# iamgroot42/A-LINK

Measured on AMD Instinct MI355X. Metric: 112x112 face embeddings/sec (IR-ResNet-100 ArcFace, 512-d, L2-normalised), higher is better.
Workload: dtype bf16

## Files before the change

a-link_amd/csrc/conv_igemm.hip:

```cpp
#include "conv_device.h"

namespace alink {

namespace {

template <typename T, int WP, int WC, bool DMA, bool SP>
__global__ __launch_bounds__(256, 2) void conv_igemm_kernel(const ConvParams p) {
    typedef typename Vec8<T>::type vec8;
    constexpr int BM = WP * 64, BN = WC * 64;
    constexpr int PJ = BM / 32, WJ = BN / 32;
    constexpr int TILE_BYTES = (BM + BN) * 128;
    extern __shared__ __attribute__((aligned(16))) char smem[];

    const int tid  = threadIdx.x;
    const int lane = tid & 63;
    const int wave = __builtin_amdgcn_readfirstlane(tid >> 6);
    const int wp = wave / WC, wc = wave % WC;

    const int ntn = p.Cout / BN;
    const int nwg = gridDim.x;
    const int lid = xcd_remap(blockIdx.x, nwg);
    const int tile_n = lid % ntn, tile_m = lid / ntn;
    const int m0 = tile_m * BM, n0 = tile_n * BN;
    const int split = blockIdx.y;

    const int Cin = p.Cin, W = p.W, ksz = p.ksz;
    const int CinP = SP ? 2 * Cin : Cin;
    const int Cin2 = SP ? 0 : p.Cin2;
    const int K = (SP ? 2 : 1) * ksz * ksz * Cin + Cin2;
    const int cpt = Cin >> 6;
    const int cpt2 = Cin2 >> 6;
    const int ntap = ksz * ksz;
    const int nk = ntap * cpt * (SP ? 3 : 1) + cpt2;
    const int kt0 = split * p.ksteps_per_split;
    const int kt1 = min(kt0 + p.ksteps_per_split, nk);

    const T* __restrict__ gin = (const T*)p.in;
    const T* __restrict__ gin2 = (const T*)p.in2;
    const T* __restrict__ gw  = (const T*)p.wgt;
    const T* __restrict__ gz  = (const T*)p.zero;

    const int chunk = (tid & 7) ^ ((tid >> 4) & 7);
    int      poff[PJ], poff2[PJ];
    unsigned pmask[PJ];
    {
        const int HoWo = p.Ho * p.Wo;
#pragma unroll
        for (int j = 0; j < PJ; ++j) {
            const int m = m0 + (tid >> 3) + 32 * j;
            unsigned mask = 0;
            int off = 0;
            poff2[j] = -1;
            if (m < p.M) {
                const int n = m / HoWo, rem = m - n * HoWo;
                const int oy = rem / p.Wo, ox = rem - oy * p.Wo;
                const int iy0 = oy * p.stride - p.pad, ix0 = ox * p.stride - p.pad;
                off = ((n * p.H + iy0) * W + ix0) * CinP + chunk * 8;
                poff2[j] = (p.in2_compact ? m : (n * p.H + oy * p.stride) * W + ox * p.stride) * Cin2 + chunk * 8;
                for (int ky = 0; ky < ksz; ++ky)
                    for (int kx = 0; kx < ksz; ++kx)
                        if ((unsigned)(iy0 + ky) < (unsigned)p.H && (unsigned)(ix0 + kx) < (unsigned)W)
                            mask |= 1u << (ky * ksz + kx);
            }
            poff[j] = off;
            pmask[j] = mask;
        }
    }
    int woff[WJ];
#pragma unroll
    for (int j = 0; j < WJ; ++j) woff[j] = (n0 + (tid >> 3) + 32 * j) * K + chunk * 8;

    const int r0 = SP ? kt0 / 3 : kt0;
    int s_ph = SP ? kt0 - 3 * r0 : 0;
    int s_tap = r0 / cpt, s_cc = r0 - s_tap * cpt;
    int s_ky = s_tap / ksz, s_kx = s_tap - s_ky * ksz;

    auto stage = [&](int buf, int kt) {
        char* base = smem + buf * TILE_BYTES;
        const int tap_off = (s_ky * W + s_kx) * CinP + (SP ? 2 * s_cc + (s_ph == 2 ? 1 : 0) : s_cc) * 64;
        const int wk_off = SP ? ((s_tap * cpt + s_cc) * 2 + (s_ph == 1 ? 1 : 0)) * 64 : kt * 64;
        const bool shortcut = !SP && s_tap == ntap;
#pragma unroll
        for (int j = 0; j < PJ; ++j) {
            const bool ok = shortcut ? poff2[j] >= 0 : (pmask[j] >> s_tap) & 1u;
            const T* src = ok ? (shortcut ? gin2 + (poff2[j] + s_cc * 64) : gin + (poff[j] + tap_off)) : gz + (tid & 7) * 8;
            if constexpr (DMA) {
                dma16(src, base + (wave * 8 + 32 * j) * 128);
            } else {
                *(uint4*)(base + ((tid >> 3) + 32 * j) * 128 + (tid & 7) * 16) = *(const uint4*)src;
            }
        }
        char* wbase = base + BM * 128;
#pragma unroll
        for (int j = 0; j < WJ; ++j) {
            const T* src = gw + (woff[j] + wk_off);
            if constexpr (DMA) {
                dma16(src, wbase + (wave * 8 + 32 * j) * 128);
            } else {
                *(uint4*)(wbase + ((tid >> 3) + 32 * j) * 128 + (tid & 7) * 16) = *(const uint4*)src;
            }
        }
        if (SP && ++s_ph < 3) return;
        s_ph = 0;
        if (++s_cc == (shortcut ? cpt2 : cpt)) {
            s_cc = 0;
            ++s_tap;
            if (++s_kx == ksz) { s_kx = 0; ++s_ky; }
        }
    };

    const int q = lane >> 4, lr = lane & 15;
    const int sw = lr >> 1;
    const int foff0 = lr * 128 + (((0 | q) ^ sw) << 4);
    const int foff1 = lr * 128 + (((4 | q) ^ sw) << 4);

    f32x4 acc[4][4];
#pragma unroll
    for (int t = 0; t < 4; ++t)
#pragma unroll
        for (int u = 0; u < 4; ++u) acc[t][u] = f32x4{0.f, 0.f, 0.f, 0.f};

    auto mma = [&](const char* pb, const char* wb) {
#pragma unroll
        for (int ks = 0; ks < 2; ++ks) {
            const int fo = ks ? foff1 : foff0;
            vec8 wf[4], pf[4];
#pragma unroll
            for (int t = 0; t < 4; ++t) wf[t] = *(const vec8*)(wb + t * 2048 + fo);
#pragma unroll
            for (int u = 0; u < 4; ++u) pf[u] = *(const vec8*)(pb + u * 2048 + fo);
#pragma unroll
            for (int t = 0; t < 4; ++t)
#pragma unroll
                for (int u = 0; u < 4; ++u) acc[t][u] = mfma16<T>(wf[t], pf[u], acc[t][u]);
        }
    };
    if constexpr (SP) {
        char* const A0 = smem, * const W0 = smem + BM * 128, * const A1 = smem + TILE_BYTES, * const W1 = smem + TILE_BYTES + BM * 128;
        auto stage_a = [&](char* dst, int part) {
            const int tap_off = (s_ky * W + s_kx) * CinP + (2 * s_cc + part) * 64;
#pragma unroll
            for (int j = 0; j < PJ; ++j) {
                const bool ok = (pmask[j] >> s_tap) & 1u;
                dma16(ok ? gin + (poff[j] + tap_off) : gz + (tid & 7) * 8, dst + (wave * 8 + 32 * j) * 128);
            }
        };
        auto stage_w = [&](char* dst, int blk) {
            const int wk_off = ((s_tap * cpt + s_cc) * 2 + blk) * 64;
#pragma unroll
            for (int j = 0; j < WJ; ++j) dma16(gw + (woff[j] + wk_off), dst + (wave * 8 + 32 * j) * 128);
        };
        auto advance = [&]() {
            if (++s_cc == cpt) {
                s_cc = 0;
                ++s_tap;
                if (++s_kx == ksz) { s_kx = 0; ++s_ky; }
            }
        };
        const int r1 = kt1 / 3;
        if (p.nprod == 1) {
            if (r0 < r1) {
                stage_a(A1, 0);
                stage_w(W0, 0);
                __syncthreads();
                for (int r = r0; r < r1; ++r) {
                    const bool odd = (r - r0) & 1;
                    advance();
                    if (r + 1 < r1) {
                        stage_a(odd ? A1 : A0, 0);
                        stage_w(odd ? W0 : W1, 0);
                    }
                    mma((odd ? A0 : A1) + (wp * 64) * 128, (odd ? W1 : W0) + (wc * 64) * 128);
                    __syncthreads();
                }
            }
        } else
        if (r0 < r1) {
            stage_a(A0, 1);
            stage_w(W0, 0);
            __syncthreads();
            const char* const pa0 = A0 + (wp * 64) * 128, * const pa1 = A1 + (wp * 64) * 128;
            const char* const pw0 = W0 + (wc * 64) * 128, * const pw1 = W1 + (wc * 64) * 128;
            for (int r = r0; r < r1; ++r) {
                stage_a(A1, 0);
                mma(pa0, pw0);
                __syncthreads();
                stage_w(W1, 1);
                mma(pa1, pw0);
                __syncthreads();
                advance();
                if (r + 1 < r1) {
                    stage_a(A0, 1);
                    stage_w(W0, 0);
                }
                mma(pa1, pw1);
                __syncthreads();
            }
        }
    } else
    if (kt0 < kt1) {
        stage(0, kt0);
        __syncthreads();
        for (int kt = kt0; kt < kt1; ++kt) {
            const int cur = (kt - kt0) & 1;
            if (kt + 1 < kt1) stage(cur ^ 1, kt + 1);
            mma(smem + cur * TILE_BYTES + (wp * 64) * 128, smem + cur * TILE_BYTES + (BM + wc * 64) * 128);
            __syncthreads();
        }
    }

    const int cbase = n0 + wc * 64 + 16 * q;
    if (p.splitk > 1) {
        float* slab = (float*)p.out + (size_t)split * p.M * p.Cout;
#pragma unroll
        for (int u = 0; u < 4; ++u) {
            const int m = m0 + wp * 64 + 16 * u + lr;
            if (m < p.M) {
                float* o = slab + (size_t)m * p.Cout + cbase;
#pragma unroll
                for (int t = 0; t < 4; ++t) *(f32x4*)(o + 4 * t) = acc[t][u];
            }
        }
        return;
    }

    const int HoWo = p.Ho * p.Wo;
    size_t off[4];
    bool ok[4];
    int cls[4];
#pragma unroll
    for (int u = 0; u < 4; ++u) {
        const int m = m0 + wp * 64 + 16 * u + lr;
        ok[u] = m < p.M;
        const int mc = ok[u] ? m : p.M - 1;
        off[u] = SP ? (size_t)mc * (2 * p.Cout) + (size_t)(cbase >> 6) * 128 + (cbase & 63) : (size_t)mc * p.Cout + cbase;
        cls[u] = 0;
        if (p.border_cls) {
            const int rem = mc % HoWo;
            const int oy = rem / p.Wo, ox = rem - oy * p.Wo;
            const int rc = (oy == 0) ? 0 : ((oy == p.Ho - 1) ? 2 : 1);
            const int cc = (ox == 0) ? 0 : ((ox == p.Wo - 1) ? 2 : 1);
            cls[u] = rc * 3 + cc;
        }
    }
    vec8 res[4][SP ? 4 : 2];
    const T* extra = (const T*)(p.dact ? p.dact : p.resid);
    if (extra) {
#pragma unroll
        for (int u = 0; u < 4; ++u) {
            res[u][0] = *(const vec8*)(extra + off[u]);
            res[u][1] = *(const vec8*)(extra + off[u] + 8);
            if (SP) {
                res[u][2] = *(const vec8*)(extra + off[u] + 64);
                res[u][3] = *(const vec8*)(extra + off[u] + 72);
            }
        }
    }
    f32x4 bia[4][4];
#pragma unroll
    for (int u = 0; u < 4; ++u)
#pragma unroll
        for (int t = 0; t < 4; ++t) bia[u][t] = *(const f32x4*)(p.bias + cls[u] * p.Cout + cbase + 4 * t);
    float al[16];
    if (p.alpha) {
#pragma unroll
        for (int t = 0; t < 4; ++t) {
            const f32x4 a4 = *(const f32x4*)(p.alpha + cbase + 4 * t);
#pragma unroll
            for (int j = 0; j < 4; ++j) al[4 * t + j] = a4[j];
        }
    }
#pragma unroll
    for (int u = 0; u < 4; ++u) {
        float v[16];
#pragma unroll
        for (int t = 0; t < 4; ++t)
#pragma unroll
            for (int j = 0; j < 4; ++j)
                v[4 * t + j] = SP ? fmaf(acc[t][u][j], p.acc_scale, bia[u][t][j] * p.bias_scale) : acc[t][u][j] + bia[u][t][j];
        if (!SP && p.dact) {
#pragma unroll
            for (int i = 0; i < 8; ++i) {
                v[i] *= (float)res[u][0][i] > 0.f ? 1.f : al[i];
                v[8 + i] *= (float)res[u][1][i] > 0.f ? 1.f : al[8 + i];
            }
        } else {
            if (p.alpha) {
#pragma unroll
                for (int i = 0; i < 16; ++i) v[i] = v[i] > 0.f ? v[i] : v[i] * al[i];
            }
            if (p.resid) {
#pragma unroll
                for (int i = 0; i < 8; ++i) {
                    if (SP) {
                        v[i] = fmaf((float)res[u][0][i] + (float)res[u][2][i], p.res_scale, v[i]);
                        v[8 + i] = fmaf((float)res[u][1][i] + (float)res[u][3][i], p.res_scale, v[8 + i]);
                    } else {
                        v[i] += (float)res[u][0][i];
                        v[8 + i] += (float)res[u][1][i];
                    }
                }
            }
        }
        if (p.post_relu) {
#pragma unroll
            for (int i = 0; i < 16; ++i) v[i] = relu_keep_nan(v[i]);
        }
        if (ok[u]) {
            vec8 o0, o1;
#pragma unroll
            for (int i = 0; i < 8; ++i) {
                o0[i] = (T)v[i];
                o1[i] = (T)v[8 + i];
            }
            *(vec8*)((T*)p.out + off[u]) = o0;
            *(vec8*)((T*)p.out + off[u] + 8) = o1;
            if (SP) {
                vec8 l0, l1;
#pragma unroll
                for (int i = 0; i < 8; ++i) {
                    l0[i] = (T)(v[i] - (float)o0[i]);
                    l1[i] = (T)(v[8 + i] - (float)o1[i]);
                }
                *(vec8*)((T*)p.out + off[u] + 64) = l0;
                *(vec8*)((T*)p.out + off[u] + 72) = l1;
            }
        }
    }
}

template <typename T, int WP, int WC, bool DMA, bool SP = false>
hipError_t launch_one(const ConvParams& p, hipStream_t stream) {
    constexpr int BM = WP * 64, BN = WC * 64;
    constexpr size_t lds = 2 * (size_t)(BM + BN) * 128;
    const int ntm = (p.M + BM - 1) / BM, ntn = p.Cout / BN;
    dim3 grid(ntm * ntn, p.splitk, 1), block(256, 1, 1);
    hipLaunchKernelGGL((conv_igemm_kernel<T, WP, WC, DMA, SP>), grid, block, lds, stream, p);
    return hipGetLastError();
}

template <typename T, int WP, int WC, bool DMA, bool SP = false>
hipError_t set_attr_one() {
    constexpr size_t lds = 2 * (size_t)(WP * 64 + WC * 64) * 128;
    return hipFuncSetAttribute((const void*)conv_igemm_kernel<T, WP, WC, DMA, SP>,
                               hipFuncAttributeMaxDynamicSharedMemorySize, (int)lds);
}

bool g_use_dma = true;

}

extern "C" void alink_debug_set_dma(int on) { g_use_dma = on != 0; }

hipError_t conv_set_attributes() {
    hipError_t e;
#define A(T, WP, WC)                                                    \
    if ((e = set_attr_one<T, WP, WC, true>()) != hipSuccess) return e;  \
    if ((e = set_attr_one<T, WP, WC, false>()) != hipSuccess) return e;
    A(__bf16, 4, 1) A(__bf16, 2, 2) A(_Float16, 4, 1) A(_Float16, 2, 2)
#undef A
    if ((e = set_attr_one<_Float16, 4, 1, true, true>()) != hipSuccess) return e;
    if ((e = set_attr_one<_Float16, 2, 2, true, true>()) != hipSuccess) return e;
    return hipSuccess;
}

double conv_flops(const ConvParams& p) {
    return 2.0 * (double)p.M * (double)p.Cout * (double)(p.ksz * p.ksz * p.Cin + (p.in2 ? p.Cin2 : 0));
}

hipError_t launch_conv_igemm(int dtype, const ConvParams& p, hipStream_t stream) {
    if (p.Cin % 64 || p.Cout % 64 || p.M <= 0 || p.splitk < 1) return hipErrorInvalidValue;
    if (p.in2 ? (p.Cin2 <= 0 || p.Cin2 % 64 || p.splitk != 1 || dtype == ALINK_DT_F16X2) : p.Cin2 != 0) return hipErrorInvalidValue;
    if ((long long)p.N * p.H * p.W * p.Cin2 >= (1ll << 31)) return hipErrorInvalidValue;
    if (p.ksz * p.ksz > 32) return hipErrorInvalidValue;
    const int two = dtype == ALINK_DT_F16X2 ? 2 : 1;
    if ((long long)p.N * p.H * p.W * p.Cin * two >= (1ll << 31)) return hipErrorInvalidValue;
    if ((long long)p.Cout * p.ksz * p.ksz * p.Cin * two >= (1ll << 31)) return hipErrorInvalidValue;
    if (conv_gemm_lat_applies(dtype, p)) return launch_conv_gemm_lat(dtype, p, stream);
    const bool wide = (p.Cout % 128) == 0;
    if (dtype == ALINK_DT_F16X2) {
        if (p.dact || (p.splitk > 1 && p.ksteps_per_split % 3)) return hipErrorInvalidValue;
        return wide ? launch_one<_Float16, 2, 2, true, true>(p, stream) : launch_one<_Float16, 4, 1, true, true>(p, stream);
    }
#define L(T)                                                                          \
    (wide ? (g_use_dma ? launch_one<T, 2, 2, true>(p, stream)                         \
                       : launch_one<T, 2, 2, false>(p, stream))                       \
          : (g_use_dma ? launch_one<T, 4, 1, true>(p, stream)                         \
                       : launch_one<T, 4, 1, false>(p, stream)))
    if (dtype == ALINK_DT_BF16) return L(__bf16);
    if (dtype == ALINK_DT_F16) return L(_Float16);
#undef L
    return hipErrorInvalidValue;
}

}
```

include/alink_hip_debug.h:

```cpp
#ifndef ALINK_HIP_DEBUG_H
#define ALINK_HIP_DEBUG_H

#include <stddef.h>

#ifdef __cplusplus
extern "C" {
#endif

void alink_debug_set_linear(int mode);
void alink_debug_set_generic_epilogue(int on);
void alink_debug_set_direct(int on);
void alink_debug_set_pair(int on);
void alink_debug_set_c64(int on);
void alink_debug_set_s2direct(int on);
void alink_debug_set_fuse_stem(int on);
void alink_debug_set_fuse_unit(int mode);
void alink_debug_set_fuse_unit1(int mode);
void alink_debug_set_fuse_shortcut(int on);
void alink_debug_set_dma(int on);
void alink_debug_set_fine_max(int n);
void alink_debug_set_sibling_aware(int on);
void alink_debug_set_latency_form(int max_pixels);
void alink_debug_set_latency_tiles(int form);
void alink_debug_set_stagger(int n);
void alink_debug_set_early_refill(int on);
void alink_debug_set_shard_stagger(int on);

void alink_debug_set_tiny_step(int on);
void alink_debug_set_mini_step(int on);
void alink_debug_set_head_bf16_mfma(int on);

void alink_debug_set_smallres_overlap(int on);
void alink_debug_set_smallres_one_update(int on);

void alink_debug_set_stop_after(int n);
void alink_debug_set_profile_reps(int n);
void alink_debug_set_ablate(int a);
void alink_debug_set_stamps(void* dev_u64);
int alink_debug_lds_oob_probe(float* dev_out516, void* stream);
int alink_debug_linear_contract_ok(void);


struct alink_resnet50;
struct alink_backbone;
int alink_debug_resnet50_grad_cache_info(const struct alink_resnet50* r, int n_images, int index, size_t* byte_offset, int* H,
                                         int* W, int* C, char* name_buf, int name_len);
int alink_debug_backbone_grad_cache_info(const struct alink_backbone* bb, int n_images, int index, size_t* byte_offset, int* H,
                                         int* W, int* C, char* name_buf, int name_len);

#ifdef __cplusplus
}
#endif
#endif
```

Baseline: 50460.

## Add eight-wave wide-tile implicit-GEMM conv kernel with three-stage LDS pipeline

Adds a 512-thread conv kernel with 128x256 or 256x128 tiles and a configurable two- or three-stage LDS pipeline using async DMA with counted waits. It is chosen by default for Cout divisible by 256 when the grid still covers the compute units, aiming to raise operand reuse per workgroup and hide global load latency. The epilogue is factored into a templated helper with a specialised plain variant that drops unused bias-class, residual and activation logic. Optional per-block timing stamps are added too. The risks are lower occupancy (one workgroup per CU, large LDS use) and fewer workgroups on small layers.

```diff
diff --git a/a-link_amd/csrc/conv_igemm.hip b/a-link_amd/csrc/conv_igemm.hip
--- a/a-link_amd/csrc/conv_igemm.hip
+++ b/a-link_amd/csrc/conv_igemm.hip
@@ -3,6 +3,9 @@
 namespace alink {
 
 namespace {
+
+template <typename T, bool SP, int EPI>
+__device__ __forceinline__ void igemm_epilogue(const ConvParams& p, const f32x4 (&acc)[4][4], int mrow0, int cbase, int lr, int split);
 
 template <typename T, int WP, int WC, bool DMA, bool SP>
 __global__ __launch_bounds__(256, 2) void conv_igemm_kernel(const ConvParams p) {
@@ -23,6 +26,9 @@
     const int tile_n = lid % ntn, tile_m = lid / ntn;
     const int m0 = tile_m * BM, n0 = tile_n * BN;
     const int split = blockIdx.y;
+    unsigned long long* const stamps = (SP || p.splitk > 1) ? nullptr : (unsigned long long*)p.stamps;
+    unsigned long long wait_cycles = 0;
+    if (stamps && tid == 0) stamps[(size_t)blockIdx.x * 8 + 0] = __builtin_amdgcn_s_memtime();
 
     const int Cin = p.Cin, W = p.W, ksz = p.ksz;
     const int CinP = SP ? 2 * Cin : Cin;
@@ -201,20 +207,40 @@
     if (kt0 < kt1) {
         stage(0, kt0);
         __syncthreads();
+        if (stamps && tid == 0) stamps[(size_t)blockIdx.x * 8 + 1] = __builtin_amdgcn_s_memtime();
         for (int kt = kt0; kt < kt1; ++kt) {
             const int cur = (kt - kt0) & 1;
             if (kt + 1 < kt1) stage(cur ^ 1, kt + 1);
             mma(smem + cur * TILE_BYTES + (wp * 64) * 128, smem + cur * TILE_BYTES + (BM + wc * 64) * 128);
-            __syncthreads();
-        }
-    }
-
-    const int cbase = n0 + wc * 64 + 16 * q;
-    if (p.splitk > 1) {
+            if (stamps) {
+                asm volatile("s_waitcnt lgkmcnt(0)" ::: "memory");
+                const unsigned long long t0 = __builtin_amdgcn_s_memtime();
+                __syncthreads();
+                wait_cycles += __builtin_amdgcn_s_memtime() - t0;
+            } else {
+                __syncthreads();
+            }
+        }
+    }
+
+    if (stamps && tid == 0) stamps[(size_t)blockIdx.x * 8 + 2] = __builtin_amdgcn_s_memtime();
+    igemm_epilogue<T, SP, 0>(p, acc, m0 + wp * 64, n0 + wc * 64 + 16 * q, lr, split);
+    if (stamps && tid == 0) {
+        asm volatile("s_waitcnt vmcnt(0)" ::: "memory");
+        stamps[(size_t)blockIdx.x * 8 + 3] = __builtin_amdgcn_s_memtime();
+        stamps[(size_t)blockIdx.x * 8 + 4] = wait_cycles;
+        stamps[(size_t)blockIdx.x * 8 + 5] = (unsigned long long)(kt1 - kt0);
+    }
+}
+
+template <typename T, bool SP, int EPI>
+__device__ __forceinline__ void igemm_epilogue(const ConvParams& p, const f32x4 (&acc)[4][4], int mrow0, int cbase, int lr, int split) {
+    typedef typename Vec8<T>::type vec8;
+    if (EPI == 0 && p.splitk > 1) {
         float* slab = (float*)p.out + (size_t)split * p.M * p.Cout;
 #pragma unroll
         for (int u = 0; u < 4; ++u) {
-            const int m = m0 + wp * 64 + 16 * u + lr;
+            const int m = mrow0 + 16 * u + lr;
             if (m < p.M) {
                 float* o = slab + (size_t)m * p.Cout + cbase;
 #pragma unroll
@@ -230,12 +256,12 @@
     int cls[4];
 #pragma unroll
     for (int u = 0; u < 4; ++u) {
-        const int m = m0 + wp * 64 + 16 * u + lr;
+        const int m = mrow0 + 16 * u + lr;
         ok[u] = m < p.M;
         const int mc = ok[u] ? m : p.M - 1;
         off[u] = SP ? (size_t)mc * (2 * p.Cout) + (size_t)(cbase >> 6) * 128 + (cbase & 63) : (size_t)mc * p.Cout + cbase;
         cls[u] = 0;
-        if (p.border_cls) {
+        if (EPI == 0 && p.border_cls) {
             const int rem = mc % HoWo;
             const int oy = rem / p.Wo, ox = rem - oy * p.Wo;
             const int rc = (oy == 0) ? 0 : ((oy == p.Ho - 1) ? 2 : 1);
@@ -244,7 +270,7 @@
         }
     }
     vec8 res[4][SP ? 4 : 2];
-    const T* extra = (const T*)(p.dact ? p.dact : p.resid);
+    const T* extra = EPI == 0 ? (const T*)(p.dact ? p.dact : p.resid) : nullptr;
     if (extra) {
 #pragma unroll
         for (int u = 0; u < 4; ++u) {
@@ -261,8 +287,9 @@
     for (int u = 0; u < 4; ++u)
 #pragma unroll
         for (int t = 0; t < 4; ++t) bia[u][t] = *(const f32x4*)(p.bias + cls[u] * p.Cout + cbase + 4 * t);
+    const bool prelu = EPI == 0 && p.alpha;
     float al[16];
-    if (p.alpha) {
+    if (prelu) {
 #pragma unroll
         for (int t = 0; t < 4; ++t) {
             const f32x4 a4 = *(const f32x4*)(p.alpha + cbase + 4 * t);
@@ -278,18 +305,18 @@
 #pragma unroll
             for (int j = 0; j < 4; ++j)
                 v[4 * t + j] = SP ? fmaf(acc[t][u][j], p.acc_scale, bia[u][t][j] * p.bias_scale) : acc[t][u][j] + bia[u][t][j];
-        if (!SP && p.dact) {
+        if (EPI == 0 && !SP && p.dact) {
 #pragma unroll
             for (int i = 0; i < 8; ++i) {
                 v[i] *= (float)res[u][0][i] > 0.f ? 1.f : al[i];
                 v[8 + i] *= (float)res[u][1][i] > 0.f ? 1.f : al[8 + i];
             }
         } else {
-            if (p.alpha) {
+            if (prelu) {
 #pragma unroll
                 for (int i = 0; i < 16; ++i) v[i] = v[i] > 0.f ? v[i] : v[i] * al[i];
             }
-            if (p.resid) {
+            if (EPI == 0 && p.resid) {
 #pragma unroll
                 for (int i = 0; i < 8; ++i) {
                     if (SP) {
@@ -302,7 +329,7 @@
                 }
             }
         }
-        if (p.post_relu) {
+        if (EPI == 0 && p.post_relu) {
 #pragma unroll
             for (int i = 0; i < 16; ++i) v[i] = relu_keep_nan(v[i]);
         }
@@ -326,6 +353,169 @@
                 *(vec8*)((T*)p.out + off[u] + 72) = l1;
             }
         }
+    }
+}
+
+template <typename T, int WP, int WC, int STAGES, int EPI>
+__global__ __launch_bounds__(512, 1) void conv_igemm_wide_kernel(const ConvParams p) {
+    typedef typename Vec8<T>::type vec8;
+    static_assert(WP * WC == 8 && (STAGES == 2 || STAGES == 3), "eight waves, two or three LDS stages");
+    constexpr int BM = WP * 64, BN = WC * 64;
+    constexpr int PJ = BM / 64, WJ = BN / 64;
+    constexpr int NP = PJ + WJ;
+    constexpr int TILE_BYTES = (BM + BN) * 128;
+    extern __shared__ __attribute__((aligned(16))) char smem[];
+
+    const int tid  = threadIdx.x;
+    const int lane = tid & 63;
+    const int wave = __builtin_amdgcn_readfirstlane(tid >> 6);
+    const int wp = wave / WC, wc = wave % WC;
+
+    const int ntn = p.Cout / BN;
+    const int lid = xcd_remap(blockIdx.x, gridDim.x);
+    const int tile_n = lid % ntn, tile_m = lid / ntn;
+    const int m0 = tile_m * BM, n0 = tile_n * BN;
+    unsigned long long* const stamps = EPI == 1 ? nullptr : (unsigned long long*)p.stamps;
+    unsigned long long wait_cycles = 0;
+    if (stamps && tid == 0) stamps[(size_t)blockIdx.x * 8 + 0] = __builtin_amdgcn_s_memtime();
+
+    const int Cin = p.Cin, W = p.W, ksz = p.ksz;
+    const int Cin2 = p.Cin2;
+    const int K = ksz * ksz * Cin + Cin2;
+    const int cpt = Cin >> 6, cpt2 = Cin2 >> 6;
+    const int ntap = ksz * ksz;
+    const int nk = ntap * cpt + cpt2;
+
+    const unsigned long long gin = (unsigned long long)p.in, gin2 = (unsigned long long)p.in2;
+    const char* gw = (const char*)p.wgt;
+
+    const int chunk = (tid & 7) ^ ((tid >> 4) & 7);
+    const unsigned long long gzl = (unsigned long long)p.zero + (tid & 7) * 16;
+    unsigned poff[PJ], poff2[PJ], pmask[PJ];
+    {
+        const int HoWo = p.Ho * p.Wo;
+#pragma unroll
+        for (int j = 0; j < PJ; ++j) {
+            const int m = m0 + (tid >> 3) + 64 * j;
+            unsigned mask = 0;
+            poff[j] = poff2[j] = 0;
+            if (m < p.M) {
+                const int n = m / HoWo, rem = m - n * HoWo;
+                const int oy = rem / p.Wo, ox = rem - oy * p.Wo;
+                const int iy0 = oy * p.stride - p.pad, ix0 = ox * p.stride - p.pad;
+                poff[j] = (unsigned)(((n * p.H + iy0) * W + ix0) * Cin + chunk * 8) * 2u;
+                poff2[j] = (unsigned)((p.in2_compact ? m : (n * p.H + oy * p.stride) * W + ox * p.stride) * Cin2 + chunk * 8) * 2u;
+                mask = 1u << ntap;
+                for (int ky = 0; ky < ksz; ++ky)
+                    for (int kx = 0; kx < ksz; ++kx)
+                        if ((unsigned)(iy0 + ky) < (unsigned)p.H && (unsigned)(ix0 + kx) < (unsigned)W)
+                            mask |= 1u << (ky * ksz + kx);
+            }
+            pmask[j] = mask;
+        }
+    }
+    unsigned woff[WJ];
+#pragma unroll
+    for (int j = 0; j < WJ; ++j) woff[j] = (unsigned)((n0 + (tid >> 3) + 64 * j) * K + chunk * 8) * 2u;
+
+    struct Cursor { int tap, cc, ky, kx; };
+    Cursor cs = {0, 0, 0, 0};
+    const char* gwk = gw;
+    auto next = [=](Cursor c) {
+        if (c.tap == ntap) { ++c.cc; return c; }
+        if (++c.cc == cpt) {
+            c.cc = 0;
+            ++c.tap;
+            if (++c.kx == ksz) { c.kx = 0; ++c.ky; }
+        }
+        return c;
+    };
+    auto stage = [&](int buf, const Cursor c, const char* wk) {
+        char* base = smem + buf * TILE_BYTES;
+        char* wbase = base + BM * 128;
+#pragma unroll
+        for (int j = 0; j < WJ; ++j) dma16(wk + woff[j], wbase + (wave * 8 + 64 * j) * 128);
+        if (c.tap == ntap) {
+            const unsigned sadd = (unsigned)c.cc * 128u;
+#pragma unroll
+            for (int j = 0; j < PJ; ++j) {
+                const bool ok = (pmask[j] >> c.tap) & 1u;
+                dma16((const void*)(ok ? gin2 + (poff2[j] + sadd) : gzl), base + (wave * 8 + 64 * j) * 128);
+            }
+        } else {
+            const unsigned sadd = (unsigned)((c.ky * W + c.kx) * Cin + c.cc * 64) * 2u;
+#pragma unroll
+            for (int j = 0; j < PJ; ++j) {
+                const bool ok = (pmask[j] >> c.tap) & 1u;
+                dma16((const void*)(ok ? gin + (poff[j] + sadd) : gzl), base + (wave * 8 + 64 * j) * 128);
+            }
+        }
+    };
+
+    const int q = lane >> 4, lr = lane & 15;
+    const int sw = lr >> 1;
+    const int foff0 = lr * 128 + (((0 | q) ^ sw) << 4);
+    const int foff1 = lr * 128 + (((4 | q) ^ sw) << 4);
+
+    f32x4 acc[4][4];
+#pragma unroll
+    for (int t = 0; t < 4; ++t)
+#pragma unroll
+        for (int u = 0; u < 4; ++u) acc[t][u] = f32x4{0.f, 0.f, 0.f, 0.f};
+
+    auto mma = [&](const char* pb, const char* wb) {
+#pragma unroll
+        for (int ks = 0; ks < 2; ++ks) {
+            const int fo = ks ? foff1 : foff0;
+            vec8 wf[4], pf[4];
+#pragma unroll
+            for (int t = 0; t < 4; ++t) wf[t] = *(const vec8*)(wb + t * 2048 + fo);
+#pragma unroll
+            for (int u = 0; u < 4; ++u) pf[u] = *(const vec8*)(pb + u * 2048 + fo);
+#pragma unroll
+            for (int t = 0; t < 4; ++t)
+#pragma unroll
+                for (int u = 0; u < 4; ++u) acc[t][u] = mfma16<T>(wf[t], pf[u], acc[t][u]);
+        }
+    };
+
+    stage(0, cs, gwk);
+    cs = next(cs); gwk += 128;
+    if (STAGES == 3 && nk > 1) {
+        stage(1, cs, gwk);
+        cs = next(cs); gwk += 128;
+        wait_then_barrier<NP>();
+    } else {
+        wait_then_barrier<0>();
+    }
+    if (stamps && tid == 0) stamps[(size_t)blockIdx.x * 8 + 1] = __builtin_amdgcn_s_memtime();
+    int cur = 0, nxt = STAGES - 1;
+    for (int kt = 0; kt < nk; ++kt) {
+        const bool more = kt + STAGES - 1 < nk;
+        if (more) {
+            stage(nxt, cs, gwk);
+            cs = next(cs); gwk += 128;
+        }
+        mma(smem + cur * TILE_BYTES + (wp * 64) * 128, smem + cur * TILE_BYTES + (BM + wc * 64) * 128);
+        unsigned long long t0 = 0;
+        if (stamps) {
+            asm volatile("s_waitcnt lgkmcnt(0)" ::: "memory");
+            t0 = __builtin_amdgcn_s_memtime();
+        }
+        if (STAGES == 3 && more) wait_then_barrier<NP>();
+        else                     wait_then_barrier<0>();
+        if (stamps) wait_cycles += __builtin_amdgcn_s_memtime() - t0;
+        cur = cur + 1 == STAGES ? 0 : cur + 1;
+        nxt = nxt + 1 == STAGES ? 0 : nxt + 1;
+    }
+
+    if (stamps && tid == 0) stamps[(size_t)blockIdx.x * 8 + 2] = __builtin_amdgcn_s_memtime();
+    igemm_epilogue<T, false, EPI>(p, acc, m0 + wp * 64, n0 + wc * 64 + 16 * q, lr, 0);
+    if (stamps && tid == 0) {
+        asm volatile("s_waitcnt vmcnt(0)" ::: "memory");
+        stamps[(size_t)blockIdx.x * 8 + 3] = __builtin_amdgcn_s_memtime();
+        stamps[(size_t)blockIdx.x * 8 + 4] = wait_cycles;
+        stamps[(size_t)blockIdx.x * 8 + 5] = (unsigned long long)nk;
     }
 }
 
@@ -346,9 +536,58 @@
                                hipFuncAttributeMaxDynamicSharedMemorySize, (int)lds);
 }
 
+#ifndef ALINK_IGEMM_WIDE_STAGES
+#define ALINK_IGEMM_WIDE_STAGES 3
+#endif
+constexpr int WIDE_STAGES = ALINK_IGEMM_WIDE_STAGES;
+
+template <typename T, int WP, int WC, int EPI>
+hipError_t launch_wide(const ConvParams& p, hipStream_t stream) {
+    constexpr int BM = WP * 64, BN = WC * 64;
+    constexpr size_t lds = WIDE_STAGES * (size_t)(BM + BN) * 128;
+    dim3 grid(((p.M + BM - 1) / BM) * (p.Cout / BN), 1, 1), block(512, 1, 1);
+    hipLaunchKernelGGL((conv_igemm_wide_kernel<T, WP, WC, WIDE_STAGES, EPI>), grid, block, lds, stream, p);
+    return hipGetLastError();
+}
+
+template <typename T, int WP, int WC, int EPI>
+hipError_t set_attr_wide() {
+    constexpr size_t lds = WIDE_STAGES * (size_t)(WP * 64 + WC * 64) * 128;
+    return hipFuncSetAttribute((const void*)conv_igemm_wide_kernel<T, WP, WC, WIDE_STAGES, EPI>,
+                               hipFuncAttributeMaxDynamicSharedMemorySize, (int)lds);
+}
+
 bool g_use_dma = true;
-
-}
+int  g_igemm_wide = 1;
+
+int compute_units() {
+    static int cus[16] = {};
+    const int dev = current_device();
+    if (dev < 0 || dev >= 16) return 1 << 30;
+    if (!cus[dev] && hipDeviceGetAttribute(&cus[dev], hipDeviceAttributeMultiprocessorCount, dev) != hipSuccess) {
+        (void)hipGetLastError();
+        cus[dev] = 0;
+        return 1 << 30;
+    }
+    return cus[dev];
+}
+
+template <typename T>
+bool try_wide(const ConvParams& p, hipStream_t stream, hipError_t* e) {
+    if (!g_igemm_wide || !g_use_dma || p.dact || p.splitk != 1 || p.ksz * p.ksz >= 32) return false;
+    const bool c256 = p.Cout % 256 == 0;
+    if (!c256 && p.Cout % 128) return false;
+    const long long nwg = (long long)((p.M + (c256 ? 127 : 255)) / (c256 ? 128 : 256)) * (p.Cout / (c256 ? 256 : 128));
+    if (g_igemm_wide != 2 && (!c256 || 4 * nwg < compute_units())) return false;
+    const bool plain = !p.border_cls && !p.alpha && !p.resid && !p.post_relu && !p.stamps;
+    *e = c256 ? (plain ? launch_wide<T, 2, 4, 1>(p, stream) : launch_wide<T, 2, 4, 0>(p, stream))
+              : (plain ? launch_wide<T, 4, 2, 1>(p, stream) : launch_wide<T, 4, 2, 0>(p, stream));
+    return true;
+}
+
+}
+
+extern "C" void alink_debug_set_igemm_wide(int mode) { g_igemm_wide = mode < 0 ? 0 : (mode > 2 ? 2 : mode); }
 
 extern "C" void alink_debug_set_dma(int on) { g_use_dma = on != 0; }
 
@@ -361,6 +600,11 @@
 #undef A
     if ((e = set_attr_one<_Float16, 4, 1, true, true>()) != hipSuccess) return e;
     if ((e = set_attr_one<_Float16, 2, 2, true, true>()) != hipSuccess) return e;
+#define A(T, WP, WC)                                                    \
+    if ((e = set_attr_wide<T, WP, WC, 0>()) != hipSuccess) return e;    \
+    if ((e = set_attr_wide<T, WP, WC, 1>()) != hipSuccess) return e;
+    A(__bf16, 4, 2) A(__bf16, 2, 4) A(_Float16, 4, 2) A(_Float16, 2, 4)
+#undef A
     return hipSuccess;
 }
 
@@ -382,6 +626,8 @@
         if (p.dact || (p.splitk > 1 && p.ksteps_per_split % 3)) return hipErrorInvalidValue;
         return wide ? launch_one<_Float16, 2, 2, true, true>(p, stream) : launch_one<_Float16, 4, 1, true, true>(p, stream);
     }
+    hipError_t ew;
+    if (dtype == ALINK_DT_BF16 ? try_wide<__bf16>(p, stream, &ew) : (dtype == ALINK_DT_F16 && try_wide<_Float16>(p, stream, &ew))) return ew;
 #define L(T)                                                                          \
     (wide ? (g_use_dma ? launch_one<T, 2, 2, true>(p, stream)                         \
                        : launch_one<T, 2, 2, false>(p, stream))                       \
diff --git a/include/alink_hip_debug.h b/include/alink_hip_debug.h
--- a/include/alink_hip_debug.h
+++ b/include/alink_hip_debug.h
@@ -18,6 +18,7 @@
 void alink_debug_set_fuse_unit1(int mode);
 void alink_debug_set_fuse_shortcut(int on);
 void alink_debug_set_dma(int on);
+void alink_debug_set_igemm_wide(int mode);
 void alink_debug_set_fine_max(int n);
 void alink_debug_set_sibling_aware(int on);
 void alink_debug_set_latency_form(int max_pixels);
```

Result: no change. 50680, median of 6 (+0.4%).
